# nz0001na/MorphGANformer

Measured on AMD Instinct MI355X. Metric: latent-projection iters/sec @1024^2, k=17 latents, higher is better.
Workload: dtype f32; 1 GPU; configs[1]: single 1024x1024 face per GPU, Wing+LPIPS(squeeze)+MSE literal-mode projection step, noise_mode=random, seeded synthetic weights/targets/landmarks; k=17, z_dim=32, targets_per_gpu=1, parallelism=pair-sharded x1, graph_replay=True, loss_generator_overlap=True, steps_per_forward=32

## Files before the change

### include/mgf.h

```cpp
#ifndef MGF_H_
#define MGF_H_

#include <stdint.h>

#ifdef __cplusplus
extern "C" {
#endif

typedef void* mgf_stream_t;

enum { MGF_OK = 0, MGF_EINVAL = -1, MGF_EUNSUPPORTED = -2, MGF_ELAUNCH = -3, MGF_ETOOBIG = -4 };
enum { MGF_F32 = 0, MGF_F64 = 1, MGF_F16 = 2 };
enum { MGF_FILTER_SEPARABLE = 2 };
enum { MGF_FILTER_LARGE = 4 };
enum { MGF_ACT_LINEAR = 1, MGF_ACT_RELU = 2, MGF_ACT_LRELU = 3, MGF_ACT_TANH = 4, MGF_ACT_SIGMOID = 5,
       MGF_ACT_ELU = 6, MGF_ACT_SELU = 7, MGF_ACT_SOFTPLUS = 8, MGF_ACT_SWISH = 9,
       MGF_ACT_RELU_POST = 10 };

const char* mgf_last_error(void);
int mgf_version(void);
int mgf_device_ok(void);

int mgf_bias_act(void* y, const void* x, const void* b, const void* xref, const void* yref, const void* dy,
                 int dtype, int64_t numel, int64_t step_b, int64_t size_b,
// ... 118 lines not shown
                          int32_t n, int32_t wdim, int32_t max_cin, mgf_stream_t stream);

int mgf_duplex_attention(float* y, const float* x, const float* wqc, const float* spos, const float* vwb,
                         int32_t n, int32_t c, int32_t f, int32_t t,
                         const mgf_epilogue* ep, int32_t ep_w, float* probs, int32_t* argmax, mgf_stream_t stream);

int mgf_att_map_upsample_f32(float* out, const float* probs, int32_t n, int32_t side, int32_t t, int32_t out_res, int32_t layer,
                             int32_t n_layers, mgf_stream_t stream);

typedef struct mgf_attn_job {
    const float* wmv;
    const float* bmv;
    float* vwb;
    int32_t c;
    int32_t w_offset;
} mgf_attn_job;
int mgf_attn_values(const mgf_attn_job* job, const float* ws, int64_t ws_stride_n, int64_t ws_stride_t, int32_t n, int32_t t,
                    int32_t wdim, mgf_stream_t stream);
int mgf_attn_values_multi(const mgf_attn_job* jobs_dev, int32_t njobs, const float* ws, int64_t ws_stride_n, int64_t ws_stride_t,
                          int32_t n, int32_t t, int32_t wdim, mgf_stream_t stream);

int mgf_randn_f32(float* out, int64_t n, uint64_t seed, void* state, mgf_stream_t stream);
int mgf_rgb_weights_f32(float* out, const float* w, const float* s, int32_t n, int32_t c, int32_t cout, mgf_stream_t stream);

int64_t mgf_mapping_param_floats(int32_t k, int32_t dim, int32_t n_res_layers);
int mgf_mapping_forward(float* w, const float* z, const float* params, int32_t n, int32_t k, int32_t dim,
                        int32_t n_res_layers, int32_t normalize_global, mgf_stream_t stream);

int64_t mgf_reduce_scratch_floats(void);
int mgf_mse_f32(float* out, const float* a, const float* b, int32_t n, int64_t numel, int64_t b_batch_stride, float scale,
                int32_t accumulate, float* scratch, mgf_stream_t stream);
int64_t mgf_dssim_scratch_bytes(int32_t n, int32_t c, int32_t h, int32_t w);
int mgf_dssim_u8_f32(float* out, const float* img, const float* target, int32_t n, int32_t c, int32_t h, int32_t w, int64_t t_batch_stride,
                     float data_range, float scale, int32_t accumulate, void* scratch, mgf_stream_t stream);
int64_t mgf_lbp_scratch_bytes(int32_t n);
int mgf_lbp_gray224_u8(uint8_t* gray, const float* img, const int32_t* tables, int32_t n, int32_t h, int32_t w, int32_t true_rgb_order,
                       mgf_stream_t stream);
int mgf_lbp_codes_u8(uint8_t* codes, const uint8_t* gray, const double* offsets, int32_t n, mgf_stream_t stream);
int mgf_lbp_distance_f64(double* out, const uint8_t* gray, const uint8_t* target_codes, const double* offsets, int32_t n, void* scratch,
                         mgf_stream_t stream);
int mgf_wing_loss_f64(double* out, const double* pred, const double* target, int32_t n, int64_t numel, double omega, double epsilon,
                      const int32_t* pred_step, int32_t max_row, mgf_stream_t stream);
int mgf_adaptive_wing_loss_f64(double* out, const double* pred, const double* target, int32_t n, int64_t numel, double omega, double theta,
                               double epsilon, double alpha, const int32_t* pred_step, int32_t max_row, mgf_stream_t stream);
int mgf_lpips_unit_f32(float* out, const float* f, int32_t n, int32_t c, int64_t hw, mgf_stream_t stream);
int mgf_lpips_layer_f32(float* out, const float* f0, const float* f1_unit, const float* lin, int32_t n, int32_t c, int64_t hw,
// ... 142 lines not shown
```

### morphganformer_amd/_lib.py

```python
from __future__ import annotations

import ctypes as C
import os

import torch

HERE = os.path.dirname(os.path.abspath(__file__))
LIB_PATH = os.environ.get("MGF_LIB_PATH") or os.path.join(HERE, "libmgf_hip.so")

MGF_F32, MGF_F64, MGF_F16 = 0, 1, 2
ACT_IDS = {"linear": 1, "relu": 2, "lrelu": 3, "tanh": 4, "sigmoid": 5, "elu": 6, "selu": 7, "softplus": 8, "swish": 9,
           "relu_post": 10}
MAX_TAPS = 9

i32, i64, f32, f64, vp = C.c_int32, C.c_int64, C.c_float, C.c_double, C.c_void_p


class Epilogue(C.Structure):
    _fields_ = [("bias", vp), ("noise", vp), ("noise_strength", vp), ("noise_n", i32), ("act", i32), ("alpha", f32),
                ("gain", f32), ("residual", vp)]


class ConvDesc(C.Structure):
    _fields_ = [("n", i32), ("cin", i32), ("in_h", i32), ("in_w", i32), ("cout", i32), ("cout_pad", i32),
# ... 49 lines not shown
    "mgf_conv3x3_winograd3_f32": (C.c_int, [vp, vp, vp, vp, vp, i32, i32, i32, i32, i32, i32, C.POINTER(Epilogue), vp]),
    "mgf_conv1x1_f32": (C.c_int, [vp, vp, vp, vp, i32, i32, i32, i32, i32, i64, i32, C.POINTER(Epilogue), vp]),
    "mgf_conv3x3s2_few_inputs_f32": (C.c_int, [vp, vp, vp, vp, i32, i32, i32, i32, i32, i32, vp]),
    "mgf_tconv3x3s2_few_outputs_f32": (C.c_int, [vp, vp, vp, i32, i32, i32, i32, i32, i32, i32, i64, i64, vp]),
    "mgf_conv1x1_force_shape": (C.c_int, [i32]),
    "mgf_conv3x3_winograd3_slice_f32": (C.c_int, [vp, vp, vp, vp, vp, i32, i32, i32, i32, i32, i32, i64, i32, C.POINTER(Epilogue), vp]),
    "mgf_conv3x3_winograd3_up2res_f32": (C.c_int, [vp, vp, vp, vp, vp, vp, i32, i32, i32, i32, i32, i32, C.POINTER(Epilogue), vp]),
    "mgf_winograd3_force_shape": (C.c_int, [i32]),
    "mgf_conv3x3_winograd3_rgb_f32": (C.c_int, [vp, vp, vp, vp, vp, vp, vp, i32, i32, i32, i32, i32, i32, i32, vp]),
    "mgf_conv3x3_winograd2_slice_f32": (C.c_int, [vp, vp, vp, vp, vp, i32, i32, i32, i32, i32, i32, i64, i32, C.POINTER(Epilogue), vp]),
    "mgf_pack_conv_weights": (C.c_int, [vp, vp, vp, i32, i32, i32, i32, i32, f32, i32, vp]),
    "mgf_conv_profile_begin": (C.c_int, []),
    "mgf_conv_profile_end": (C.c_int, [C.POINTER(ConvProfRec), i32]),
    "mgf_demod_f32": (C.c_int, [vp, vp, vp, i32, i32, i32, vp]),
    "mgf_demod_bwd_f32": (C.c_int, [vp, vp, vp, vp, vp, i32, i32, i32, vp]),
    "mgf_style_demod": (C.c_int, [C.POINTER(StyleJob), vp, i64, i32, i32, vp]),
    "mgf_style_demod_multi": (C.c_int, [vp, i32, vp, i64, i32, i32, i32, vp]),
    "mgf_duplex_attention": (C.c_int, [vp, vp, vp, vp, vp, i32, i32, i32, i32, C.POINTER(Epilogue), i32, vp, vp, vp]),
    "mgf_att_map_upsample_f32": (C.c_int, [vp, vp, i32, i32, i32, i32, i32, i32, vp]),
    "mgf_attn_values": (C.c_int, [C.POINTER(AttnJob), vp, i64, i64, i32, i32, i32, vp]),
    "mgf_attn_values_multi": (C.c_int, [vp, i32, vp, i64, i64, i32, i32, i32, vp]),
    "mgf_randn_f32": (C.c_int, [vp, i64, C.c_uint64, vp, vp]),
    "mgf_rgb_weights_f32": (C.c_int, [vp, vp, vp, i32, i32, i32, vp]),
    "mgf_mapping_param_floats": (i64, [i32, i32, i32]),
    "mgf_mapping_forward": (C.c_int, [vp, vp, vp, i32, i32, i32, i32, i32, vp]),
    "mgf_reduce_scratch_floats": (i64, []),
    "mgf_mse_f32": (C.c_int, [vp, vp, vp, i32, i64, i64, f32, i32, vp, vp]),
    "mgf_dssim_scratch_bytes": (i64, [i32, i32, i32, i32]),
    "mgf_dssim_u8_f32": (C.c_int, [vp, vp, vp, i32, i32, i32, i32, i64, f32, f32, i32, vp, vp]),
    "mgf_lbp_scratch_bytes": (i64, [i32]),
    "mgf_lbp_gray224_u8": (C.c_int, [vp, vp, vp, i32, i32, i32, i32, vp]),
    "mgf_lbp_codes_u8": (C.c_int, [vp, vp, vp, i32, vp]),
    "mgf_lbp_distance_f64": (C.c_int, [vp, vp, vp, vp, i32, vp, vp]),
    "mgf_wing_loss_f64": (C.c_int, [vp, vp, vp, i32, i64, f64, f64, vp, i32, vp]),
    "mgf_adaptive_wing_loss_f64": (C.c_int, [vp, vp, vp, i32, i64, f64, f64, f64, f64, vp, i32, vp]),
    "mgf_lpips_unit_f32": (C.c_int, [vp, vp, i32, i32, i64, vp]),
    "mgf_lpips_layer_f32": (C.c_int, [vp, vp, vp, vp, i32, i32, i64, i64, i32, vp, vp]),
    "mgf_lpips_stem_f32": (C.c_int, [vp, vp, vp, vp, vp, vp, vp, vp, i32, i32, i32, i32, vp, vp]),
    "mgf_channel_affine_prelu_f32": (C.c_int, [vp, vp, vp, vp, vp, i32, i32, i64, vp]),
    "mgf_linear_f32": (C.c_int, [vp, vp, vp, vp, i32, i32, i32, vp]),
    "mgf_resize_bilinear_f32": (C.c_int, [vp, vp, i32, i32, i32, i32, i32, vp]),
    "mgf_spatial_mean_f32": (C.c_int, [vp, vp, i32, i64, vp]),
    "mgf_l2_normalize_f32": (C.c_int, [vp, vp, i32, i32, f32, vp]),
    "mgf_l2_normalize_bwd_f32": (C.c_int, [vp, vp, vp, i32, i32, f32, vp]),
    "mgf_spatial_mean_bwd_f32": (C.c_int, [vp, vp, i32, i64, vp]),
    "mgf_relu_bwd_slice_f32": (C.c_int, [vp, vp, i32, i32, vp, i32, i32, i32, i32, i64, vp]),
# ... 109 lines not shown
```

### morphganformer_amd/conv.py

```python
from __future__ import annotations

import ctypes as C
import os
from dataclasses import dataclass

import torch

from . import _lib


def round_up(v: int, m: int) -> int:
    return (v + m - 1) // m * m


def profile_begin():
    _lib.check(_lib.lib().mgf_conv_profile_begin(), "conv_profile_begin")


def profile_end(max_recs=4096):
    recs = (_lib.ConvProfRec * max_recs)()
    n = _lib.lib().mgf_conv_profile_end(recs, max_recs)
    if n < 0:
        _lib.check(n, "conv_profile_end")
    return [(recs[i].kernel.decode(), recs[i].flops, recs[i].seconds, recs[i].ksplit, recs[i].bytes) for i in range(min(n, max_recs))]
# ... 337 lines not shown
TCONV_SPLIT_MIN = int(os.environ.get("MGF_TCONV_SPLIT_MIN", "16"))


def tconv_pitch(w: int, align: int = 4) -> int:
    return round_up(2 * w + 1, align)


def conv3x3s2_few_inputs(x, w, bias=None, relu=False, out=None):
    _lib.require_gpu(x, w, bias, out)
    cout, cin = w.shape[:2]
    assert tuple(w.shape[2:]) == (3, 3) and cin <= 4 and w.is_contiguous() and w.dtype == torch.float32
    assert x.dtype == torch.float32 and x.is_contiguous() and x.shape[1] == cin
    n, _, h, wd = x.shape
    oh, ow = (h - 3) // 2 + 1, (wd - 3) // 2 + 1
    if out is None:
        out = torch.empty([n, cout, oh, ow], dtype=torch.float32, device=x.device)
    assert out.is_contiguous() and tuple(out.shape) == (n, cout, oh, ow)
    rc = _lib.lib().mgf_conv3x3s2_few_inputs_f32(out.data_ptr(), x.data_ptr(), w.data_ptr(), _lib.ptr(bias), n, cin, h, wd, cout, int(relu),
                                                 _lib.stream_ptr())
    _lib.check(rc, "conv3x3s2_few_inputs")
    return out


def tconv3x3s2_forward(x, pc: PackedConv, in_scale=None, out_scale=None, out=None, bf=None):
    _lib.require_gpu(x, pc.wp, in_scale, out_scale, out)
    assert pc.kh == 3 and pc.kw == 3 and x.dtype == torch.float32 and x.is_contiguous()
    n, cin, h, w = x.shape
    oh, ow = 2 * h + 1, 2 * w + 1
    if out is None:
        out = torch.empty([n, pc.cout, oh, tconv_pitch(w)], dtype=torch.float32, device=x.device)
    pitch = out.shape[3]
    assert out.is_contiguous() and tuple(out.shape) == (n, pc.cout, oh, pitch) and pitch >= ow and pitch % 4 == 0
    if NARROW_CONV and pc.cout <= 4 and in_scale is None and out_scale is None:
        rc = _lib.lib().mgf_tconv3x3s2_few_outputs_f32(out.data_ptr(), x.data_ptr(), pc.wp.data_ptr(), n, cin, h, w, pc.cout, pc.cout_pad,
                                                       pitch, oh * pitch, pc.cout * oh * pitch, _lib.stream_ptr())
        _lib.check(rc, "tconv3x3s2_few_outputs")
        return out[:, :, :, :ow]
    split = SPLIT_TCONV_BORDER and min(h, w) >= (TCONV_SPLIT_MIN if n >= 4 else max(TCONV_SPLIT_MIN, 128))
    use_bf = bf is not None and split and w % 32 == 0 and cin % 16 == 0
    os_stride = 0 if out_scale is None else out_scale.stride(0) if out_scale.ndim == 2 else 0
    d = _desc(n, cin, h, w, pc.cout, pc.cout_pad, h if split else h + 1, w if split else w + 1, 1, 2, TCONV_TAPS, TCONV_GROUPS,
              [0, 0, 1, 1], [0, 1, 0, 1], oh, ow, pitch, oh * pitch, pc.cout * oh * pitch, 0, os_stride)
    if use_bf:
        rc = _lib.lib().mgf_conv_taps_bf16x3_f32(out.data_ptr(), x.data_ptr(), bf.data_ptr(), _lib.ptr(in_scale), _lib.ptr(out_scale),
                                                 C.byref(d), None, _lib.stream_ptr())
    else:
# ... 28 lines not shown
```

### morphganformer_amd/csrc/latent_prep.hip

```cpp
#include "mgf_common.h"

namespace {

__device__ void style_demod_body(const mgf_style_job& j, const float* ws, int64_t ws_stride_n, int wdim, int n, float* s_lds,
                                 bool styles_only = false) {
    const int tid = threadIdx.x;
    const float* wg = ws + (int64_t)n * ws_stride_n + j.w_offset;
    for (int ci = tid; ci < j.cin; ci += blockDim.x) {
        const float* row = j.aff_w + (int64_t)ci * wdim;
        float acc = 0.f;
        for (int k = 0; k < wdim; ++k) acc += wg[k] * row[k];
        float s = (acc * j.aff_gain + j.aff_b[ci]) * j.style_gain;
        s_lds[ci] = s;
        if (blockIdx.x == 0) j.s[(int64_t)n * j.cin + ci] = s;
    }
    if (!j.wsq || !j.d || styles_only) return;
    __syncthreads();
    const int lane = tid & 63, wave = tid >> 6, nwaves = blockDim.x >> 6;
    const int per_block = (j.cout + gridDim.x - 1) / gridDim.x;
    const int co_begin = blockIdx.x * per_block;
    const int co_end = min(j.cout, co_begin + per_block);
    for (int co = co_begin + wave; co < co_end; co += nwaves) {
        const float* row = j.wsq + (int64_t)co * j.cin;
        float acc = 0.f;
// ... 680 lines not shown
            float sn, cs;
            sincospif(2.f * u2, &sn, &cs);
            z[2 * h] = r * cs; z[2 * h + 1] = r * sn;
        }
        if (4 * q + 4 <= n && (((uintptr_t)out) & 15) == 0) *reinterpret_cast<float4*>(out + 4 * q) = make_float4(z[0], z[1], z[2], z[3]);
        else for (int e = 0; e < 4 && 4 * q + e < n; ++e) out[4 * q + e] = z[e];
    }
    __syncthreads();
    if (threadIdx.x == 0) {
        const unsigned prev = __hip_atomic_fetch_add(ticket, 1u, __ATOMIC_ACQ_REL, __HIP_MEMORY_SCOPE_AGENT);
        if (prev == gridDim.x - 1) {
            __hip_atomic_store(ticket, 0u, __ATOMIC_RELAXED, __HIP_MEMORY_SCOPE_AGENT);
            __hip_atomic_store(counter, base + (unsigned long long)quads, __ATOMIC_RELAXED, __HIP_MEMORY_SCOPE_AGENT);
        }
    }
}

__global__ __launch_bounds__(256) void rgb_weights_kernel(float* out, const float* w, const float* s, int c, int co, int total) {
    const int i = blockIdx.x * 256 + threadIdx.x;
    if (i >= total) return;
    const int o = i % co, n = i / (c * co);
    out[i] = w[i % (c * co)] * s[n * co + o];
}
}

extern "C" int mgf_randn_f32(float* out, int64_t n, uint64_t seed, void* state, mgf_stream_t stream) {
    MGF_REQUIRE(out && state && n >= 1, MGF_EINVAL, "randn: bad arguments");
    MGF_REQUIRE(((uintptr_t)state % 8) == 0, MGF_EINVAL, "randn: the 16-byte state {uint64 counter, uint32 ticket, pad} must be 8-byte aligned");
    const int grid = mgf_stream_grid((n + 3) / 4, 256, 4);
    hipLaunchKernelGGL(randn_kernel, dim3(grid), dim3(256), 0, (hipStream_t)stream, out, n, seed, reinterpret_cast<unsigned long long*>(state),
                       reinterpret_cast<unsigned*>(reinterpret_cast<char*>(state) + 8));
    MGF_CHECK_LAUNCH("randn");
    return MGF_OK;
}

extern "C" int mgf_rgb_weights_f32(float* out, const float* w, const float* s, int32_t n, int32_t c, int32_t cout, mgf_stream_t stream) {
    MGF_REQUIRE(out && w && s && n >= 1 && c >= 1 && cout >= 1 && (int64_t)n * c * cout <= INT32_MAX, MGF_EINVAL, "rgb_weights: bad arguments");
    const int total = n * c * cout;
    hipLaunchKernelGGL(rgb_weights_kernel, dim3((unsigned)mgf_cdiv(total, 256)), dim3(256), 0, (hipStream_t)stream, out, w, s, c, cout, total);
    MGF_CHECK_LAUNCH("rgb_weights");
    return MGF_OK;
}

extern "C" int mgf_mapping_forward_save(float* w, const float* z, const float* params, float* scratch, int32_t n, int32_t k, int32_t dim,
                                        int32_t n_res_layers, int32_t normalize_global, mgf_stream_t stream) {
    MGF_REQUIRE(w && z && params && scratch, MGF_EINVAL, "mapping_forward_save: null pointer");
    MGF_REQUIRE(dim == MD, MGF_EUNSUPPORTED, "mapping_forward_save: latent width must be %d (got %d)", MD, dim);
    MGF_REQUIRE(k >= 2 && k - 1 <= MT_MAX, MGF_EUNSUPPORTED, "mapping_forward_save: k must be in 2..%d (got %d)", MT_MAX + 1, k);
    MGF_REQUIRE(n >= 1 && n_res_layers >= 0, MGF_EINVAL, "mapping_forward_save: bad sizes");
    MGF_REQUIRE(n_res_layers <= MAP_MAX_RES, MGF_EUNSUPPORTED, "mapping_forward_save: at most %d residual layers (got %d)", MAP_MAX_RES, n_res_layers);
    hipLaunchKernelGGL(mapping_save_kernel, dim3(n, 2), dim3(MAP_BLOCK), 0, (hipStream_t)stream, w, z, params, scratch,
                       mgf_mapping_bwd_scratch_floats(k, dim, n_res_layers), k, n_res_layers, normalize_global);
    MGF_CHECK_LAUNCH("mapping_forward_save");
    return MGF_OK;
}

extern "C" int mgf_mapping_backward_saved(float* dz, const float* dw, const float* z, const float* params, float* scratch, int32_t n,
                                          int32_t k, int32_t dim, int32_t n_res_layers, int32_t normalize_global, mgf_stream_t stream) {
    MGF_REQUIRE(dz && dw && z && params && scratch, MGF_EINVAL, "mapping_backward_saved: null pointer");
    MGF_REQUIRE(dim == MD, MGF_EUNSUPPORTED, "mapping_backward_saved: latent width must be %d (got %d)", MD, dim);
    MGF_REQUIRE(k >= 2 && k - 1 <= MT_MAX, MGF_EUNSUPPORTED, "mapping_backward_saved: k must be in 2..%d (got %d)", MT_MAX + 1, k);
    MGF_REQUIRE(n >= 1 && n_res_layers >= 0, MGF_EINVAL, "mapping_backward_saved: bad sizes");
    MGF_REQUIRE(n_res_layers <= MAP_MAX_RES, MGF_EUNSUPPORTED, "mapping_backward_saved: at most %d residual layers (got %d)", MAP_MAX_RES, n_res_layers);
// ... 18 lines not shown
```

### morphganformer_amd/csrc/narrow_conv.hip

```cpp
#include "mgf_common.h"

namespace {

constexpr int NC_MAX_NARROW = 4;
constexpr int NC_MAX_WIDE = 1024;

typedef const float __attribute__((address_space(4)))* nc_cfp;

template <int CIN>
__global__ __launch_bounds__(256) void conv3x3s2_few_inputs_kernel(float* __restrict__ y, const float* __restrict__ x, const float* w,
                                                                   const float* bias, int in_h, int in_w, int cout, int out_h, int out_w,
                                                                   int relu) {
    constexpr int K = CIN * 9;
    const int n = blockIdx.z, oy = blockIdx.y, ox = blockIdx.x * 256 + threadIdx.x;
    if (ox >= out_w) return;
    float v[K];
    const float* xb = x + (int64_t)n * CIN * in_h * in_w + (int64_t)(2 * oy) * in_w + 2 * ox;
#pragma unroll
    for (int k = 0; k < K; ++k) v[k] = xb[(int64_t)(k / 9) * in_h * in_w + ((k % 9) / 3) * in_w + (k % 3)];
    float* yb = y + (int64_t)n * cout * out_h * out_w + (int64_t)oy * out_w + ox;
    const int64_t plane = (int64_t)out_h * out_w;
    const nc_cfp ws = (nc_cfp)w, bs = (nc_cfp)bias;
#ifndef MGF_NC_UNROLL
#define MGF_NC_UNROLL 2
// ... 52 lines not shown
                a10[u][o] += wt[3][o] * p + wt[5][o] * q;
                a11[u][o] += wt[4][o] * p;
            }
        }
    }
#pragma unroll
    for (int u = 0; u < 2; ++u) {
        if (u == 1 && !q1) break;
        const bool r0 = i + u < h;
        float* yb = y + (int64_t)n * y_batch + (int64_t)(2 * (i + u)) * pitch + 2 * j;
#pragma unroll
        for (int o = 0; o < CO; ++o) {
            float* yo = yb + o * y_plane;
            if (c0) *reinterpret_cast<float2*>(yo) = make_float2(a00[u][o], a01[u][o]);
            else yo[0] = a00[u][o];
            if (r0) {
                if (c0) *reinterpret_cast<float2*>(yo + pitch) = make_float2(a10[u][o], a11[u][o]);
                else yo[pitch] = a10[u][o];
            }
        }
    }
}

}

extern "C" int mgf_conv3x3s2_few_inputs_f32(float* y, const float* x, const float* w, const float* bias, int32_t n, int32_t cin, int32_t in_h,
                                            int32_t in_w, int32_t cout, int32_t relu, mgf_stream_t stream) {
    MGF_REQUIRE(y && x && w && n >= 1 && in_h >= 3 && in_w >= 3, MGF_EINVAL, "conv3x3s2_few_inputs: bad arguments");
    MGF_REQUIRE(cin >= 1 && cin <= NC_MAX_NARROW, MGF_EUNSUPPORTED, "conv3x3s2_few_inputs: 1..%d input channels (got %d)", NC_MAX_NARROW, cin);
    MGF_REQUIRE(cout >= 1, MGF_EINVAL, "conv3x3s2_few_inputs: bad channel count");
    MGF_REQUIRE(n <= 65535, MGF_ETOOBIG, "conv3x3s2_few_inputs: n must be <= 65535");
    const int out_h = (in_h - 3) / 2 + 1, out_w = (in_w - 3) / 2 + 1;
    MGF_REQUIRE((int64_t)cout * out_h * out_w <= INT32_MAX && (int64_t)cin * in_h * in_w <= INT32_MAX, MGF_ETOOBIG, "conv3x3s2_few_inputs: sample too large");
    MGF_REQUIRE(out_h <= 65535, MGF_ETOOBIG, "conv3x3s2_few_inputs: at most 65535 output rows");
    const dim3 grid((unsigned)mgf_cdiv(out_w, 256), (unsigned)out_h, n);
    hipStream_t st = (hipStream_t)stream;
#define MGF_CFI_LAUNCH(CI) \
    hipLaunchKernelGGL(conv3x3s2_few_inputs_kernel<CI>, grid, dim3(256), 0, st, y, x, w, bias, in_h, in_w, cout, out_h, out_w, relu)
    if (cin == 1) MGF_CFI_LAUNCH(1); else if (cin == 2) MGF_CFI_LAUNCH(2); else if (cin == 3) MGF_CFI_LAUNCH(3); else MGF_CFI_LAUNCH(4);
#undef MGF_CFI_LAUNCH
    MGF_CHECK_LAUNCH("conv3x3s2_few_inputs");
    return MGF_OK;
}

extern "C" int mgf_tconv3x3s2_few_outputs_f32(float* y, const float* x, const float* wp, int32_t n, int32_t cin, int32_t h, int32_t w,
                                              int32_t cout, int32_t cout_pad, int32_t pitch, int64_t y_plane, int64_t y_batch,
// ... 20 lines not shown
```

### morphganformer_amd/csrc/wino3.hip

```cpp
#include "mgf_common.h"
#include <algorithm>
#include <cstdlib>
#include <type_traits>

namespace {

typedef float f32x16 __attribute__((ext_vector_type(16)));
typedef float v2f __attribute__((ext_vector_type(2)));

struct Wino3Params {
    float* y;
    const float* x;
    const float* u;
    const float* in_scale;
    const float* out_scale;
    int n, cin, h, w, cout, os_stride;
    int tiles_x, tiles_y, co_tiles;
    int xcd_per;
    mgf_epilogue ep;
    int has_ep;
    const float* rgb_w;
    const float* rgb_bias;
    float* rgb_out;
    int rgb_channels;
// ... 463 lines not shown
                 : "memory");
}

__device__ __forceinline__ void w3_dma_b128(w3_v4i rsrc, unsigned lds_addr, unsigned voff, unsigned soff) {
    unsigned keep;
    asm volatile("s_nop 4\n\ts_mov_b32 %0, m0\n\ts_mov_b32 m0, %3\n\ts_nop 0\n\tbuffer_load_dwordx4 %1, %2, %4 offen lds\n\ts_mov_b32 m0, %0"
                 : "=&s"(keep)
                 : "v"(voff), "s"(rsrc), "s"(lds_addr), "s"(soff)
                 : "memory");
}

#ifndef W3P_XD_PLAIN
#define W3P_XD_PLAIN 4
#endif
#ifndef W3P_XD_RGB
#define W3P_XD_RGB 8
#endif
template <int NCK, bool RGB>
__global__ __launch_bounds__(256, 2) void wino3p_conv_kernel(Wino3Params p) {
    static_assert(NCK % 2 == 0 && NCK >= 4, "the staging buffers alternate per chunk");
    constexpr int FP = 6 * W3FW;
    constexpr int CST = 256, RAW = W3CK * CST;
    constexpr int NV = 16, NR = 8;
    constexpr unsigned OOB = 0xFFFFFFF0u;
    extern __shared__ float lds[];
    float* const raw0 = lds;
    float* const raw1 = raw0 + RAW;
    float* const xch = raw1 + RAW;
    float* const lowt = xch + 6 * NV * 64;
    float* const nzs = lowt + 3072;
    float* const obs = nzs + 256;
    const int tid = threadIdx.x, lane = tid & 63;
    const int a = __builtin_amdgcn_readfirstlane(tid >> 6);
    const int l31 = lane & 31, half = lane >> 5;
    const int tx = l31 & 15, ty = l31 >> 4;

    int b_ = blockIdx.x;
    if (p.xcd_per > 0) {
        b_ = (b_ & 7) * p.xcd_per + (b_ >> 3);
        if (b_ >= p.n * p.strips_x * p.strips_y * p.co_tiles) return;
    }
    const int cot = b_ % p.co_tiles; b_ /= p.co_tiles;
    const int sx = b_ % p.strips_x; b_ /= p.strips_x;
    const int sy = b_ % p.strips_y;
    const int n = b_ / p.strips_y;
    const int vert = p.vert;
// ... 507 lines not shown
```

### morphganformer_amd/engine.py

```python
from __future__ import annotations

import ctypes as C
import math
import os
from dataclasses import dataclass, field

import numpy as np
import torch

from . import _lib
from . import conv as cv
from .synth_weights import GeneratorConfig

SQRT2 = math.sqrt(2.0)
SQRT_HALF = math.sqrt(0.5)
USE_WINOGRAD = os.environ.get("MGF_WINOGRAD", "1") != "0"
WINOGRAD_MAX_RES = int(os.environ.get("MGF_WINOGRAD_MAX_RES", "1024"))
BF_DIRECT_MAX_RES = int(os.environ.get("MGF_BF_DIRECT_MAX_RES", "128"))


def pack_mapping_params(sd, cfg: GeneratorConfig) -> np.ndarray:
    D, T = cfg.w_dim, cfg.k - 1
    lr = cfg.mapping_lrmul
    n_res = cfg.mapping_layers // 2
# ... 30 lines not shown
    return blob


@dataclass
class ConvLayerPlan:
    name: str
    res: int
    cin: int
    cout: int
    up: int
    slot: int
    kind: str
    pc: cv.PackedConv = None
    aff_w: torch.Tensor = None
    aff_b: torch.Tensor = None
    style_gain: float = 1.0
    demod: bool = True
    bias: torch.Tensor = None
    noise_const: torch.Tensor = None
    noise_strength: torch.Tensor = None
    act_gain: float = 1.0
    attn: "AttnPlan" = None
    w_raw: torch.Tensor = None
    wino_u: torch.Tensor = None
    pcb: torch.Tensor = None
    s_off: int = 0
    d_off: int = 0


@dataclass
class AttnPlan:
    c: int
    f: int
    wqc: torch.Tensor
    spos: torch.Tensor
    wmv: torch.Tensor
    bmv: torch.Tensor
    v_off: int = 0


class SynthesisPlan:

    def __init__(self, sd, cfg: GeneratorConfig, device="cuda", arith="f32"):
        _lib.lib()
        self.cfg = cfg
        self.arith = arith
# ... 19 lines not shown
                lp.pc = cv.pack_weights(t32(w), gain=1.0, flip=False)
                lp.w_raw = t32(w.reshape(cout, cin))
                lp.style_gain = 1.0 / math.sqrt(cin)
                lp.demod = False
            else:
                wg = 1.0 / math.sqrt(cin * 9)
                lp.pc = cv.pack_weights(t32(w), gain=wg, flip=False, want_wsq=True)
                if kind == "conv3" and USE_WINOGRAD and cv.winograd_ok(cin, cout, res, res) and res <= WINOGRAD_MAX_RES:
                    lp.wino_u = cv.winograd_pack(t32(w), wg, res)
                if arith == "bf16x3" and cin % 16 == 0 and res // up >= 32:
                    lp.pcb = cv.pack_weights_bf16x3(lp.pc)
            lp.aff_w = t32(f64(p + ".affine.weight"))
            lp.aff_b = t32(f64(p + ".affine.bias"))
            if (p + ".biasAct.bias") in sd:
                lp.bias = t32(f64(p + ".biasAct.bias"))
            if (p + ".noise_strength") in sd:
                lp.noise_strength = t32(f64(p + ".noise_strength").reshape(1))
                lp.noise_const = t32(f64(p + ".noise_const"))
            lp.act_gain = SQRT2 * (SQRT_HALF if (name == "conv1" and res > 4) else 1.0)
            if att and (p + ".transformer.to_queries.weight") in sd:
                lp.attn = self._fold_attention(sd, p, cout, res, T, D, t32, f64)
                lp.attn.v_off = v_off
                v_off += cout * T
            lp.s_off, lp.d_off = s_off, d_off
            s_off += cin
            d_off += cout
            self.layers.append(lp)
        self.s_total, self.d_total, self.v_total = s_off, d_off, v_off
        for res in cfg.block_resolutions[1:]:
            w = f64(f"synthesis.b{res}.skip.weight")
            self.skips[res] = cv.pack_weights(t32(w), gain=SQRT_HALF / math.sqrt(w.shape[1]), flip=False)
        torch.cuda.synchronize(dev)

    @staticmethod
    def _fold_attention(sd, p, C_, res, T, D, t32, f64):
        tp = p + ".transformer"
        Fn = res * res
        wq = f64(tp + ".to_queries.weight") / math.sqrt(C_)
        bq = f64(tp + ".to_queries.bias")
        wfp = f64(tp + ".from_pos_map.weight") / math.sqrt(D)
        bfp = f64(tp + ".from_pos_map.bias")
        wv = f64(tp + ".to_values.weight") / math.sqrt(D)
        bv = f64(tp + ".to_values.bias")
        wm = f64(tp + ".modulation.weight") / math.sqrt(C_)
        bm = f64(tp + ".modulation.bias")
        aw = f64(tp + ".att_weight").reshape(2 * C_)
# ... 13 lines not shown

    def __init__(self, sd, cfg: GeneratorConfig, device="cuda", max_batch: int = 1, arith: str = "f32"):
        if arith not in ("f32", "bf16x3"):
            raise ValueError(f"arith must be 'f32' or 'bf16x3' (got {arith!r})")
        self.cfg = cfg
        self.arith = arith
        self.tpitch_align = 32 if arith == "bf16x3" else 4
        self.plan = SynthesisPlan(sd, cfg, device, arith=arith)
        self.device = self.plan.device
        self.input_shape = [None, cfg.k, cfg.z_dim]
        self.cond_shape = [None, 0]
        self.z_dim, self.w_dim, self.k, self.c_dim = cfg.z_dim, cfg.w_dim, cfg.k, 0
        self.img_resolution, self.img_channels = cfg.img_resolution, cfg.img_channels
        self.num_ws = cfg.num_ws
        self.w_avg = torch.as_tensor(np.asarray(sd["mapping.w_avg"], dtype=np.float32), device=self.device)
        self._ws_cache = {}
        self.taps = None
        self.fuse_torgb = True
        self.skip_fused = {}
        self.fuse_skip_up = os.environ.get("MGF_FUSE_SKIP_UP", "1") != "0"
        self.last_noise = ("none", None)
        self.side = torch.cuda.Stream(device=self.device)
        self.overlap_skip = os.environ.get("MGF_OVERLAP_SKIP", "0") != "0"
        self._workspaces, self._pins = {}, {}
        self.noise_seed, self._noise_epoch = int(torch.initial_seed()) & 0xFFFFFFFFFFFFFFFF, None
        self.noise_state = torch.zeros(2, dtype=torch.int64, device=self.device)
        self._alloc(max_batch)

    _WS_FIELDS = ("n", "lean", "w_buf", "styles", "demods", "vtabs", "noise_rand", "bufs", "img", "const_in", "rgbw", "style_jobs", "n_style_jobs",
                  "max_style_cin", "attn_jobs", "n_attn_jobs", "style_jobs_pl", "attn_jobs_pl", "ws_bytes", "ws_gen")

    def _alloc(self, n, lean=None):
        cur = (getattr(self, "n", None), getattr(self, "lean", False))
        lean = cur[1] if lean is None else bool(lean)
        if cur[0] is not None and cur in self._workspaces:
            self._workspaces[cur]["noise_rand"] = self.noise_rand
        key = (n, lean)
        ws = self._workspaces.pop(key, None)
        if ws is None:
            self._evict_for(n, lean)
            self._create(n, lean)
            ws = {k: getattr(self, k) for k in self._WS_FIELDS}
        self._workspaces[key] = ws
        for k, v in ws.items():
            setattr(self, k, v)

    def pin(self, key=None):
        key = (self.n, self.lean) if key is None else key
        self._pins[key] = self._pins.get(key, 0) + 1
        return key

    def unpin(self, key):
# ... 79 lines not shown
                    if not self._fuses_skip_up(conv1[res], n):
                        b["skip"] = view("S", n, c, res, res)
                if res == cfg.img_resolution:
                    b["last"] = view("T", n, c, res, res)
                self.bufs[res] = b
        for res in ([] if lean else cfg.block_resolutions):
            c = cfg.channels(res)
            b = {"conv1": e(n, c, res, res)}
            if res > 4:
                b["skip_low"] = e(n, c, res // 2, res // 2)
                b["skip"] = e(n, c, res, res)
                b["t"] = e(n, c, res + 1, cv.tconv_pitch(res // 2, self.tpitch_align))
                b["conv0"] = e(n, c, res, res)
                if cfg.has_attention(res):
                    b["conv0a"] = e(n, c, res, res)
            if cfg.has_attention(res):
                b["conv1a"] = e(n, c, res, res)
            if res == cfg.img_resolution:
                b["last"] = e(n, c, res, res)
            self.bufs[res] = b
        self.img = e(n, cfg.img_channels, cfg.img_resolution, cfg.img_resolution)
        self.const_in = P.const.unsqueeze(0).repeat(n, 1, 1, 1).contiguous()
        self.rgbw = e(n, cfg.img_channels, cfg.channels(cfg.img_resolution))
        self.ws_bytes = self._workspace_bytes(n, lean)
        self._build_jobs(n)

    def _build_jobs(self, n):
        cfg, P = self.cfg, self.plan
        D, NW = cfg.w_dim, cfg.num_ws

        def tables(per_layer):
            sj = (_lib.StyleJob * len(P.layers))()
            aj = []
            for i, lp in enumerate(P.layers):
                g_off = ((cfg.k - 1) * NW + lp.slot) * D if per_layer else (cfg.k - 1) * D
                sj[i] = _lib.StyleJob(lp.aff_w.data_ptr(), lp.aff_b.data_ptr(), _lib.ptr(lp.pc.wsq) if lp.demod else 0,
                                      self.styles.data_ptr() + 4 * lp.s_off * n,
                                      (self.demods.data_ptr() + 4 * lp.d_off * n) if lp.demod else 0,
                                      lp.cin, lp.cout, g_off, 1.0 / math.sqrt(D), lp.style_gain)
                if lp.attn is not None:
                    aj.append(_lib.AttnJob(lp.attn.wmv.data_ptr(), lp.attn.bmv.data_ptr(),
                                           self.vtabs.data_ptr() + 4 * lp.attn.v_off * n, lp.attn.c, lp.slot * D if per_layer else 0))
            sjt = torch.frombuffer(bytearray(bytes(sj)), dtype=torch.uint8).to(self.device)
            ajt = None
            if aj:
                arr = (_lib.AttnJob * len(aj))(*aj)
# ... 130 lines not shown
                main = torch.cuda.current_stream(self.device)
                if self.overlap_skip:
                    self.side.wait_stream(main)
                    with torch.cuda.stream(self.side):
                        cv.conv_forward(x, P.skips[res], out=B["skip_low"])
                        if not fuse_up:
                            cv.upfirdn_into(B["skip"], B["skip_low"], P.fir, up=2, pad=(2, 1, 2, 1), gain=4.0, separable=True)
                else:
                    cv.conv_forward(x, P.skips[res], out=B["skip_low"])
                    if not fuse_up:
                        cv.upfirdn_into(B["skip"], B["skip_low"], P.fir, up=2, pad=(2, 1, 2, 1), gain=4.0, separable=True)
                x0 = self._layer(layers[b + ".conv0"], x, B, "conv0", noise_mode, noises, residual=None)
                if self.overlap_skip:
                    main.wait_stream(self.side)
                if fuse_up:
                    x = self._layer(l1, x0, B, "conv1", noise_mode, noises, residual=None, residual_low=B["skip_low"])
                else:
                    x = self._layer(l1, x0, B, "conv1", noise_mode, noises, residual=B["skip"])
            if self.taps is not None:
                self.taps[b] = x
            if res == cfg.img_resolution:
                lp = layers[b + ".conv_last"]
                lt = layers[b + ".torgb"]
                if self.taps is None and self.fuse_torgb and lp.cout <= 32:
                    _lib.check(L.mgf_rgb_weights_f32(self.rgbw.data_ptr(), lt.w_raw.data_ptr(), self._s(lt).data_ptr(), n, lt.w_raw.shape[0],
                                                     lt.w_raw.shape[1], st), "rgb_weights")
                    if lp.wino_u is not None and lp.wino_u.ndim == 4 and lp.cout == 32 and cv.winograd_fills_chip(n, lp.cout, res, res):
                        cv.winograd2_rgb_forward(x, lp.wino_u, self.rgbw, lt.bias, self.img, in_scale=self._s(lp), out_scale=self._d(lp))
                    else:
                        cv.conv_forward(x, lp.pc, pad=(1, 1), in_scale=self._s(lp), out_scale=self._d(lp),
                                        rgb=(self.rgbw, lt.bias, self.img))
                else:
                    if lp.wino_u is not None and cv.winograd_fills_chip(n, lp.cout, res, res):
                        x = cv.winograd_forward(x, lp.wino_u, in_scale=self._s(lp), out_scale=self._d(lp), out=B["last"])
                    else:
                        x = cv.conv_forward(x, lp.pc, pad=(1, 1), in_scale=self._s(lp), out_scale=self._d(lp), out=B["last"])
                    if self.taps is not None:
                        self.taps[b] = x
                    ep = _lib.make_epilogue(bias=lt.bias)
                    cv.conv_forward(x, lt.pc, in_scale=self._s(lt), epilogue=ep, out=self.img)
        return self.img

    def list2tensor(self, att_maps=None):
        att_maps = self.att_maps if att_maps is None else att_maps
        if not att_maps:
            return torch.zeros([1], device=self.device)
        T, R = self.cfg.k - 1, self.cfg.img_resolution
# ... 127 lines not shown
```

Before: 730.9 iters/s.

## Compose conv_last and ToRGB weights into a single few-output 3x3 conv

When conv_last has no bias, noise or attention, its modulated and demodulated 3x3 weights are folded with the 1x1 ToRGB weights into one effective 3x3 kernel per sample. The image is then produced by a new direct conv kernel that writes only 3 output channels. This skips materialising the 32-channel 1024x1024 intermediate and the winograd plus fused-RGB path. It adds a small double-precision weight-composition kernel and relies on conv_last being linear, which the new guard conditions check.

After: 762.9 iters/s (median of 6 runs). 4.4% higher.

```diff
diff --git a/include/mgf.h b/include/mgf.h
--- a/include/mgf.h
+++ b/include/mgf.h
@@ -164,6 +164,10 @@
 
 int mgf_randn_f32(float* out, int64_t n, uint64_t seed, void* state, mgf_stream_t stream);
 int mgf_rgb_weights_f32(float* out, const float* w, const float* s, int32_t n, int32_t c, int32_t cout, mgf_stream_t stream);
+int mgf_torgb_compose_weights_f32(float* w_eff, const float* w_last, const float* s_last, const float* d_last, const float* w_rgb,
+                                  const float* s_rgb, int32_t n, int32_t cin, int32_t cout, int32_t rgb_channels, mgf_stream_t stream);
+int mgf_conv3x3_few_outputs_f32(float* y, const float* x, const float* w, const float* bias, int32_t n, int32_t cin, int32_t h, int32_t wd,
+                                int32_t cout, mgf_stream_t stream);
 
 int64_t mgf_mapping_param_floats(int32_t k, int32_t dim, int32_t n_res_layers);
 int mgf_mapping_forward(float* w, const float* z, const float* params, int32_t n, int32_t k, int32_t dim,
diff --git a/morphganformer_amd/_lib.py b/morphganformer_amd/_lib.py
--- a/morphganformer_amd/_lib.py
+++ b/morphganformer_amd/_lib.py
@@ -95,6 +95,8 @@
     "mgf_attn_values_multi": (C.c_int, [vp, i32, vp, i64, i64, i32, i32, i32, vp]),
     "mgf_randn_f32": (C.c_int, [vp, i64, C.c_uint64, vp, vp]),
     "mgf_rgb_weights_f32": (C.c_int, [vp, vp, vp, i32, i32, i32, vp]),
+    "mgf_torgb_compose_weights_f32": (C.c_int, [vp, vp, vp, vp, vp, vp, i32, i32, i32, i32, vp]),
+    "mgf_conv3x3_few_outputs_f32": (C.c_int, [vp, vp, vp, vp, i32, i32, i32, i32, i32, vp]),
     "mgf_mapping_param_floats": (i64, [i32, i32, i32]),
     "mgf_mapping_forward": (C.c_int, [vp, vp, vp, i32, i32, i32, i32, i32, vp]),
     "mgf_reduce_scratch_floats": (i64, []),
diff --git a/morphganformer_amd/conv.py b/morphganformer_amd/conv.py
--- a/morphganformer_amd/conv.py
+++ b/morphganformer_amd/conv.py
@@ -383,6 +383,20 @@
     return out
 
 
+def conv3x3_few_outputs(x, w, bias=None, out=None):
+    _lib.require_gpu(x, w, bias, out)
+    n, cin, h, wd = x.shape
+    cout = w.shape[1]
+    assert x.dtype == torch.float32 and x.is_contiguous() and w.dtype == torch.float32 and w.is_contiguous()
+    assert tuple(w.shape) == (n, cout, cin, 3, 3) and cout <= 4
+    if out is None:
+        out = torch.empty([n, cout, h, wd], dtype=torch.float32, device=x.device)
+    assert out.is_contiguous() and tuple(out.shape) == (n, cout, h, wd)
+    _lib.check(_lib.lib().mgf_conv3x3_few_outputs_f32(out.data_ptr(), x.data_ptr(), w.data_ptr(), _lib.ptr(bias), n, cin, h, wd, cout,
+                                                      _lib.stream_ptr()), "conv3x3_few_outputs")
+    return out
+
+
 def tconv3x3s2_forward(x, pc: PackedConv, in_scale=None, out_scale=None, out=None, bf=None):
     _lib.require_gpu(x, pc.wp, in_scale, out_scale, out)
     assert pc.kh == 3 and pc.kw == 3 and x.dtype == torch.float32 and x.is_contiguous()
diff --git a/morphganformer_amd/csrc/latent_prep.hip b/morphganformer_amd/csrc/latent_prep.hip
--- a/morphganformer_amd/csrc/latent_prep.hip
+++ b/morphganformer_amd/csrc/latent_prep.hip
@@ -726,6 +726,20 @@
     const int o = i % co, n = i / (c * co);
     out[i] = w[i % (c * co)] * s[n * co + o];
 }
+
+__global__ __launch_bounds__(256) void torgb_compose_kernel(float* out, const float* w_last, const float* s_last, const float* d_last,
+                                                            const float* w_rgb, const float* s_rgb, int cin, int cout, int rc, int total) {
+    const int i = blockIdx.x * 256 + threadIdx.x;
+    if (i >= total) return;
+    const int k = i % 9, ci = (i / 9) % cin, c = (i / (9 * cin)) % rc, n = i / (9 * cin * rc);
+    double acc = 0.0;
+    for (int o = 0; o < cout; ++o) {
+        const double a = (double)w_rgb[c * cout + o] * (double)s_rgb[(int64_t)n * cout + o];
+        const double d = d_last ? (double)d_last[(int64_t)n * cout + o] : 1.0;
+        acc += a * d * (double)w_last[((int64_t)o * cin + ci) * 9 + k];
+    }
+    out[i] = (float)(acc * (double)s_last[(int64_t)n * cin + ci]);
+}
 }
 
 extern "C" int mgf_randn_f32(float* out, int64_t n, uint64_t seed, void* state, mgf_stream_t stream) {
@@ -743,6 +757,19 @@
     const int total = n * c * cout;
     hipLaunchKernelGGL(rgb_weights_kernel, dim3((unsigned)mgf_cdiv(total, 256)), dim3(256), 0, (hipStream_t)stream, out, w, s, c, cout, total);
     MGF_CHECK_LAUNCH("rgb_weights");
+    return MGF_OK;
+}
+
+extern "C" int mgf_torgb_compose_weights_f32(float* w_eff, const float* w_last, const float* s_last, const float* d_last, const float* w_rgb,
+                                             const float* s_rgb, int32_t n, int32_t cin, int32_t cout, int32_t rgb_channels, mgf_stream_t stream) {
+    MGF_REQUIRE(w_eff && w_last && s_last && w_rgb && s_rgb && n >= 1 && cin >= 1 && cout >= 1 && rgb_channels >= 1, MGF_EINVAL,
+                "torgb_compose_weights: bad arguments");
+    MGF_REQUIRE((int64_t)n * rgb_channels * cin * 9 <= INT32_MAX && (int64_t)cout * cin * 9 <= INT32_MAX, MGF_ETOOBIG,
+                "torgb_compose_weights: too many weights");
+    const int total = n * rgb_channels * cin * 9;
+    hipLaunchKernelGGL(torgb_compose_kernel, dim3((unsigned)mgf_cdiv(total, 256)), dim3(256), 0, (hipStream_t)stream, w_eff, w_last, s_last,
+                       d_last, w_rgb, s_rgb, cin, cout, rgb_channels, total);
+    MGF_CHECK_LAUNCH("torgb_compose_weights");
     return MGF_OK;
 }
 
diff --git a/morphganformer_amd/csrc/narrow_conv.hip b/morphganformer_amd/csrc/narrow_conv.hip
--- a/morphganformer_amd/csrc/narrow_conv.hip
+++ b/morphganformer_amd/csrc/narrow_conv.hip
@@ -1,3 +1,5 @@
+#include <algorithm>
+
 #include "mgf_common.h"
 
 namespace {
@@ -98,6 +100,114 @@
     }
 }
 
+typedef float nc_f2 __attribute__((ext_vector_type(2)));
+
+template <int CO, bool VEC>
+__global__ __launch_bounds__(256) void conv3x3_few_outputs_kernel(float* __restrict__ y, const float* __restrict__ x, const float* w,
+                                                                  const float* bias, int cin, int h, int wd, int rows) {
+    const int n = blockIdx.z, oy0 = blockIdx.y * rows, ox = (blockIdx.x * blockDim.x + threadIdx.x) * 4;
+    if (ox >= wd) return;
+    const int oy1 = min(oy0 + rows, h);
+    const int64_t plane = (int64_t)h * wd;
+    const float* xn = x + (int64_t)n * cin * plane + ox;
+    float* yn = y + (int64_t)n * CO * plane + ox;
+    const nc_cfp wn = (nc_cfp)w + (int64_t)n * CO * cin * 9, bs = (nc_cfp)bias;
+    nc_f2 acc[3][CO][2];
+#pragma unroll
+    for (int s = 0; s < 3; ++s)
+#pragma unroll
+        for (int o = 0; o < CO; ++o) acc[s][o][0] = acc[s][o][1] = nc_f2{0.f, 0.f};
+    for (int r = oy0 - 1; r <= oy1; ++r) {
+        if (r >= 0 && r < h) {
+            const float* xr = xn + (int64_t)r * wd;
+#ifndef MGF_C3F_UNROLL
+#define MGF_C3F_UNROLL 2
+#endif
+#pragma unroll MGF_C3F_UNROLL
+            for (int ci = 0; ci < cin; ++ci) {
+                const float* xc = xr + ci * plane;
+                float v[6];
+                if (VEC) {
+                    const float4 m = *reinterpret_cast<const float4*>(xc);
+                    v[0] = ox > 0 ? xc[-1] : 0.f;
+                    v[1] = m.x; v[2] = m.y; v[3] = m.z; v[4] = m.w;
+                    v[5] = ox + 4 < wd ? xc[4] : 0.f;
+                } else {
+#pragma unroll
+                    for (int j = 0; j < 6; ++j) v[j] = (ox + j - 1 >= 0 && ox + j - 1 < wd) ? xc[j - 1] : 0.f;
+                }
+                nc_f2 p[5];
+#pragma unroll
+                for (int k = 0; k < 5; ++k) p[k] = nc_f2{v[k], v[k + 1]};
+#pragma unroll
+                for (int kh = 0; kh < 3; ++kh)
+#pragma unroll
+                    for (int o = 0; o < CO; ++o) {
+                        const nc_cfp wr = wn + (o * cin + ci) * 9 + kh * 3;
+#pragma unroll
+                        for (int kw = 0; kw < 3; ++kw) {
+                            const float wv = wr[kw];
+                            acc[2 - kh][o][0] = __builtin_elementwise_fma(nc_f2{wv, wv}, p[kw], acc[2 - kh][o][0]);
+                            acc[2 - kh][o][1] = __builtin_elementwise_fma(nc_f2{wv, wv}, p[2 + kw], acc[2 - kh][o][1]);
+                        }
+                    }
+            }
+        }
+        if (r - 1 >= oy0) {
+            float* yr = yn + (int64_t)(r - 1) * wd;
+#pragma unroll
+            for (int o = 0; o < CO; ++o) {
+                const float b = bias ? bs[o] : 0.f;
+                const float4 q = make_float4(acc[0][o][0].x + b, acc[0][o][0].y + b, acc[0][o][1].x + b, acc[0][o][1].y + b);
+                float* yo = yr + o * plane;
+                if (VEC) {
+                    *reinterpret_cast<float4*>(yo) = q;
+                } else {
+                    yo[0] = q.x;
+                    if (ox + 1 < wd) yo[1] = q.y;
+                    if (ox + 2 < wd) yo[2] = q.z;
+                    if (ox + 3 < wd) yo[3] = q.w;
+                }
+            }
+        }
+#pragma unroll
+        for (int o = 0; o < CO; ++o)
+#pragma unroll
+            for (int u = 0; u < 2; ++u) {
+                acc[0][o][u] = acc[1][o][u];
+                acc[1][o][u] = acc[2][o][u];
+                acc[2][o][u] = nc_f2{0.f, 0.f};
+            }
+    }
+}
+
+}
+
+extern "C" int mgf_conv3x3_few_outputs_f32(float* y, const float* x, const float* w, const float* bias, int32_t n, int32_t cin, int32_t h,
+                                           int32_t wd, int32_t cout, mgf_stream_t stream) {
+    MGF_REQUIRE(y && x && w && n >= 1 && cin >= 1 && h >= 1 && wd >= 1, MGF_EINVAL, "conv3x3_few_outputs: bad arguments");
+    MGF_REQUIRE(cout >= 1 && cout <= NC_MAX_NARROW, MGF_EUNSUPPORTED, "conv3x3_few_outputs: 1..%d output channels (got %d)", NC_MAX_NARROW, cout);
+    MGF_REQUIRE(n <= 65535 && (int64_t)cout * cin * 9 <= INT32_MAX, MGF_ETOOBIG, "conv3x3_few_outputs: tensor too large");
+    const int lanes = (int)mgf_cdiv(wd, 4);
+    const int threads = (int)std::min<int64_t>(256, mgf_cdiv(lanes, MGF_WAVE) * MGF_WAVE);
+    const int gx = (int)mgf_cdiv(lanes, threads);
+    int rows = 16;
+    while (rows > 4 && (int64_t)n * gx * mgf_cdiv(h, rows) < 8 * MGF_NUM_CU) rows /= 2;
+    static const char* rows_env = mgf_knob("MGF_C3F_ROWS");
+    if (rows_env) rows = std::max(1, atoi(rows_env));
+    MGF_REQUIRE(mgf_cdiv(h, rows) <= 65535, MGF_ETOOBIG, "conv3x3_few_outputs: map too tall");
+    const bool vec = wd % 4 == 0 && ((uintptr_t)x % 16) == 0 && ((uintptr_t)y % 16) == 0;
+    const dim3 grid((unsigned)gx, (unsigned)mgf_cdiv(h, rows), (unsigned)n);
+    hipStream_t st = (hipStream_t)stream;
+#define MGF_C3F_LAUNCH(CO)                                                                                                         \
+    do {                                                                                                                           \
+        if (vec) hipLaunchKernelGGL((conv3x3_few_outputs_kernel<CO, true>), grid, dim3(threads), 0, st, y, x, w, bias, cin, h, wd, rows);  \
+        else hipLaunchKernelGGL((conv3x3_few_outputs_kernel<CO, false>), grid, dim3(threads), 0, st, y, x, w, bias, cin, h, wd, rows);     \
+    } while (0)
+    if (cout == 1) MGF_C3F_LAUNCH(1); else if (cout == 2) MGF_C3F_LAUNCH(2); else if (cout == 3) MGF_C3F_LAUNCH(3); else MGF_C3F_LAUNCH(4);
+#undef MGF_C3F_LAUNCH
+    MGF_CHECK_LAUNCH("conv3x3_few_outputs");
+    return MGF_OK;
 }
 
 extern "C" int mgf_conv3x3s2_few_inputs_f32(float* y, const float* x, const float* w, const float* bias, int32_t n, int32_t cin, int32_t in_h,
diff --git a/morphganformer_amd/csrc/wino3.hip b/morphganformer_amd/csrc/wino3.hip
--- a/morphganformer_amd/csrc/wino3.hip
+++ b/morphganformer_amd/csrc/wino3.hip
@@ -509,6 +509,7 @@
     constexpr int FP = 6 * W3FW;
     constexpr int CST = 256, RAW = W3CK * CST;
     constexpr int NV = 16, NR = 8;
+    static_assert(!RGB || NCK == NR, "the deferred ToRGB projection runs one part per chunk body and stores after part NR - 1");
     constexpr unsigned OOB = 0xFFFFFFF0u;
     extern __shared__ float lds[];
     float* const raw0 = lds;
diff --git a/morphganformer_amd/engine.py b/morphganformer_amd/engine.py
--- a/morphganformer_amd/engine.py
+++ b/morphganformer_amd/engine.py
@@ -76,6 +76,7 @@
     act_gain: float = 1.0
     attn: "AttnPlan" = None
     w_raw: torch.Tensor = None
+    w_gained: torch.Tensor = None
     wino_u: torch.Tensor = None
     pcb: torch.Tensor = None
     s_off: int = 0
@@ -141,6 +142,8 @@
                 lp.attn = self._fold_attention(sd, p, cout, res, T, D, t32, f64)
                 lp.attn.v_off = v_off
                 v_off += cout * T
+            if name == "conv_last" and lp.bias is None and lp.noise_strength is None and lp.attn is None and cfg.img_channels <= 4:
+                lp.w_gained = t32(w / math.sqrt(cin * 9))
             lp.s_off, lp.d_off = s_off, d_off
             s_off += cin
             d_off += cout
@@ -200,12 +203,13 @@
         self.last_noise = ("none", None)
         self.side = torch.cuda.Stream(device=self.device)
         self.overlap_skip = os.environ.get("MGF_OVERLAP_SKIP", "0") != "0"
+        self.torgb_compose = os.environ.get("MGF_TORGB_COMPOSE", "1") != "0"
         self._workspaces, self._pins = {}, {}
         self.noise_seed, self._noise_epoch = int(torch.initial_seed()) & 0xFFFFFFFFFFFFFFFF, None
         self.noise_state = torch.zeros(2, dtype=torch.int64, device=self.device)
         self._alloc(max_batch)
 
-    _WS_FIELDS = ("n", "lean", "w_buf", "styles", "demods", "vtabs", "noise_rand", "bufs", "img", "const_in", "rgbw", "style_jobs", "n_style_jobs",
+    _WS_FIELDS = ("n", "lean", "w_buf", "styles", "demods", "vtabs", "noise_rand", "bufs", "img", "const_in", "rgbw", "w_eff", "style_jobs", "n_style_jobs",
                   "max_style_cin", "attn_jobs", "n_attn_jobs", "style_jobs_pl", "attn_jobs_pl", "ws_bytes", "ws_gen")
 
     def _alloc(self, n, lean=None):
@@ -331,6 +335,7 @@
         self.img = e(n, cfg.img_channels, cfg.img_resolution, cfg.img_resolution)
         self.const_in = P.const.unsqueeze(0).repeat(n, 1, 1, 1).contiguous()
         self.rgbw = e(n, cfg.img_channels, cfg.channels(cfg.img_resolution))
+        self.w_eff = e(n, cfg.img_channels, cfg.channels(cfg.img_resolution), 3, 3)
         self.ws_bytes = self._workspace_bytes(n, lean)
         self._build_jobs(n)
 
@@ -507,7 +512,12 @@
             if res == cfg.img_resolution:
                 lp = layers[b + ".conv_last"]
                 lt = layers[b + ".torgb"]
-                if self.taps is None and self.fuse_torgb and lp.cout <= 32:
+                if self.taps is None and self.fuse_torgb and self.torgb_compose and lp.w_gained is not None:
+                    _lib.check(L.mgf_torgb_compose_weights_f32(self.w_eff.data_ptr(), lp.w_gained.data_ptr(), self._s(lp).data_ptr(),
+                                                               self._d(lp).data_ptr(), lt.w_raw.data_ptr(), self._s(lt).data_ptr(), n, lp.cin,
+                                                               lp.cout, lt.w_raw.shape[0], st), "torgb_compose_weights")
+                    cv.conv3x3_few_outputs(x, self.w_eff, lt.bias, out=self.img)
+                elif self.taps is None and self.fuse_torgb and lp.cout <= 32:
                     _lib.check(L.mgf_rgb_weights_f32(self.rgbw.data_ptr(), lt.w_raw.data_ptr(), self._s(lt).data_ptr(), n, lt.w_raw.shape[0],
                                                      lt.w_raw.shape[1], st), "rgb_weights")
                     if lp.wino_u is not None and lp.wino_u.ndim == 4 and lp.cout == 32 and cv.winograd_fills_chip(n, lp.cout, res, res):
```
